# JuliaLinearAlgebra/AlgebraicMultigrid.jl

Measured on AMD Instinct MI355X. Metric: V-cycle unknowns/sec + fine-level SpMV GB/s (% HBM peak), 3-D Poisson 256^3, higher is better.
Workload: dtype f64

## Files before the change

algebraicmultigrid.jl_amd/csrc/hip/amghip.hip:

```cpp
#include "amghip_internal.hpp"
#include "gs_schedule.hpp"
#include "csr_ops.hpp"
#include "chebyshev.hpp"
#include "gmres_kernels.hpp"
#include "pcg_block_kernels.hpp"
#include "dist_pcg_kernels.hpp"

namespace {

constexpr int64_t kGraphAutoRows = 65536;

struct Level {
  int64_t n = 0, nc = 0;
  amgh_csr A, S, P, R;
  bool has_S = false;
  amgh_smoother_t pre{}, post{};
  real *res = nullptr, *cx = nullptr, *cb = nullptr, *tmp = nullptr;
  real* cheb_d = nullptr;
  ChebSide cheb[2];
  const ChebSide& cheb_of(const amgh_smoother_t& s) const { return &s == &post ? cheb[1] : cheb[0]; }
  real* il = nullptr;
  amgh_csr* smat() { return has_S ? &S : &A; }
  amgh_csr Pp, Rp;
  bool lo_ok = false;
// ... 1289 lines not shown
      }
      if (L->Pp.cc.ccol) {
        double t_il = 0, t_st = 0;
        RC_TRY(hipMemsetAsync(L->cx, 0, sizeof(real) * nc * bs, h->stream) == hipSuccess ? AMGH_OK : -1001);
        RC_TRY(hipMemsetAsync(L->res, 0, sizeof(real) * n * bs, h->stream) == hipSuccess ? AMGH_OK : -1001);
        RC_TRY(timed([&] { return il_apply(bs, true, L->Pp.rowptr, L->Pp.col, L->Pp.val, n, L->cx, nc, nc, L->il, L->res, n, h->stream, &L->Pp.cc); }, &t_il));
        RC_TRY(timed([&] { return raw_apply(M_ADD, L->Pp.rowptr, L->Pp.col, L->Pp.val, n, L->cx, nc, nullptr, 0, L->res, n, h->stream, bs, &L->Pp.cc); }, &t_st));
        L->p_stream = t_st < 0.95 * t_il;
        if (getenv("AMGH_VERBOSE")) fprintf(stderr, "[amghip] n=%lld prolongation of %d columns: interleaved %.3f ms, column by column %.3f ms\n", (long long)n, bs, t_il / 2, t_st / 2);
      }
    }
  }
  if (h->nrhs == 1)
    for (Level* L : h->levels) {
      if (!L->lo_ok || !L->Rp.rowptr || L->Rp.nrows < (1 << 18)) continue;
      if (hipMemsetAsync(L->res, 0, sizeof(real) * L->n, h->stream) != hipSuccess) return -1001;
      double ms[2] = {0, 0};
      int rc = AMGH_OK;
      for (int v = 0; v < 2 && rc == AMGH_OK; ++v) {
        L->Rp.xcd_map = v == 1;
        rc = csr_apply(&L->Rp, M_SPMV, L->res, nullptr, L->cb, h->stream, 1);
        if (rc == AMGH_OK && hipEventRecord(h->t0, h->stream) != hipSuccess) rc = -1001;
        for (int r = 0; r < 4 && rc == AMGH_OK; ++r) rc = csr_apply(&L->Rp, M_SPMV, L->res, nullptr, L->cb, h->stream, 1);
        float t = 0.f;
        if (rc == AMGH_OK && (hipEventRecord(h->t1, h->stream) != hipSuccess || hipEventSynchronize(h->t1) != hipSuccess ||
                              hipEventElapsedTime(&t, h->t0, h->t1) != hipSuccess)) rc = -1001;
        ms[v] = t;
      }
      L->Rp.xcd_map = false;
      RC_TRY(rc);
      L->Rp.xcd_map = ms[1] < 0.93 * ms[0];
      if (getenv("AMGH_VERBOSE")) fprintf(stderr, "[amghip] n=%lld restriction: %.3f ms, XCD-contiguous %.3f ms -> %s\n", (long long)L->n, ms[0] / 4, ms[1] / 4, L->Rp.xcd_map ? "XCD-contiguous" : "plain");
    }
  if (gs_trim() && g_stream_code && g_trim_coded) {
    HIP_TRY(hipStreamSynchronize(h->stream));
    for (Level* L : h->levels) {
      for (amgh_csr* M : {&L->Rp, &L->Pp})
        if (M->cc.ccol && M->col && M->val) {
          hipFree(M->col); hipFree(M->val); M->col = nullptr; M->val = nullptr;
          M->bytes -= M->nnz * kEntB;
        }
      amgh_csr* S = L->smat();
      GsSchedule* g = S->gs;
      if (L->lo_cc.ccol && g && g->bw.on && g->bw.flow.on && !g->bw.rec && g->segs.empty() && !g->mf && !g->mb && g->col && g->val) {
        hipFree(g->col); hipFree(g->val); g->col = nullptr; g->val = nullptr;
        int64_t freed = g->nnz * kEntB;
        if (L->lo_val) { hipFree(L->lo_val); L->lo_val = nullptr; }
        g->csr_bytes -= freed; g->bytes -= freed; S->bytes -= freed;
      }
    }
  }
  for (size_t l = 0; l + 1 < h->levels.size(); ++l)
    if (h->levels[l]->coarse_lo) RC_TRY(gs_ensure_cols(h->levels[l + 1]->smat(), h->nrhs, h->stream));
  const int64_t n = fine_n(h);
  if (h->levels.empty()) { RC_TRY(dev_alloc(&h->res_final, n * h->nrhs)); ws += kRealB * n * h->nrhs; }
  RC_TRY(dev_alloc(&h->partial, kRedBlocks));
  RC_TRY(dev_alloc(&h->scal, 8));
  RC_TRY(dev_alloc(&h->x0, n * h->nrhs));
  RC_TRY(dev_alloc(&h->b0, n * h->nrhs));
  ws += 2 * kRealB * n * h->nrhs;
  h->ws_bytes = ws;
  if (h->graph_auto && !h->levels.empty() && getenv("AMGH_GRAPH_AUTO") && getenv("AMGH_GRAPH_AUTO")[0] == '1') {
    int64_t widest = 0;
    for (Level* L : h->levels) widest = std::max(widest, L->n);
    h->use_graph = widest <= kGraphAutoRows;
  }
// ... 504 lines not shown
}

int amgh_csr_create(amgh_csr_t** opp, int device, int64_t nrows, int64_t ncols, const int32_t* rowptr,
                    const int32_t* col, const real* val) {
  if (!opp) return AMGH_EINVAL;
  *opp = nullptr;
  int ndev = 0;
  HIP_TRY(hipGetDeviceCount(&ndev));
  if (device < 0 || device >= ndev) return AMGH_EINVAL;
  HIP_TRY(hipSetDevice(device));
  amgh_csr* op = new amgh_csr;
  int rc = csr_upload(op, device, nrows, ncols, rowptr, col, val);
  if (rc != AMGH_OK) { csr_free(op); delete op; return rc; }
  *opp = op;
  return AMGH_OK;
}
void amgh_csr_destroy(amgh_csr_t* op) {
  if (!op) return;
  hipSetDevice(op->device);
  csr_free(op);
  delete op;
}
int amgh_csr_prepare(amgh_csr_t* op, int jacobi, int gs) {
  if (!op) return AMGH_EINVAL;
  HIP_TRY(hipSetDevice(op->device));
  if (jacobi) RC_TRY(csr_ensure_diag(op, nullptr));
  if (gs) RC_TRY(csr_ensure_gs(op));
  HIP_TRY(hipDeviceSynchronize());
  return AMGH_OK;
}
int amgh_csr_spmv_d(amgh_csr_t* op, const real* x_d, real* y_d, void* stream) {
  if (!op || !x_d || !y_d) return AMGH_EINVAL;
  HIP_TRY(hipSetDevice(op->device));
  return csr_apply(op, M_SPMV, x_d, nullptr, y_d, (hipStream_t)stream);
}
int amgh_csr_residual_d(amgh_csr_t* op, const real* x_d, const real* b_d, real* r_d, void* stream) {
  if (!op || !x_d || !b_d || !r_d) return AMGH_EINVAL;
  HIP_TRY(hipSetDevice(op->device));
  return csr_apply(op, M_RESID, x_d, b_d, r_d, (hipStream_t)stream);
}
int amgh_csr_spmv_add_d(amgh_csr_t* op, const real* x_d, real* y_d, void* stream) {
  if (!op || !x_d || !y_d) return AMGH_EINVAL;
  HIP_TRY(hipSetDevice(op->device));
  return csr_apply(op, M_ADD, x_d, nullptr, y_d, (hipStream_t)stream);
}
int amgh_csr_jacobi_d(amgh_csr_t* op, double omega, const real* xin_d, const real* b_d, real* xout_d,
                      void* stream) {
  if (!op || !xin_d || !b_d || !xout_d || xin_d == xout_d) return AMGH_EINVAL;
  HIP_TRY(hipSetDevice(op->device));
  return csr_jacobi(op, omega, xin_d, b_d, xout_d, (hipStream_t)stream);
}
int amgh_csr_gs_d(amgh_csr_t* op, int backward, double omega, int is_sor, real* x_d, const real* b_d,
                  void* stream) {
  if (!op || !x_d || !b_d) return AMGH_EINVAL;
  HIP_TRY(hipSetDevice(op->device));
  return csr_gs_sweep(op, backward != 0, is_sor != 0, omega, x_d, b_d, (hipStream_t)stream);
}
int amgh_csr_gs_ex_d(amgh_csr_t* op, int backward, double omega, int is_sor, real* x_d, const real* b_d,
                     void* stream, int flags) {
  if (!op || !x_d || !b_d || (flags & ~AMGH_GS_REUSE_B)) return AMGH_EINVAL;
  HIP_TRY(hipSetDevice(op->device));
  return csr_gs_sweep(op, backward != 0, is_sor != 0, omega, x_d, b_d, (hipStream_t)stream, true, true, 1, false,
                      (flags & AMGH_GS_REUSE_B) != 0);
}

int amgh_gather_d(int device, int64_t n, const int32_t* idx_d, const real* src_d, real* dst_d, void* stream) {
  if (n < 0 || (n > 0 && (!idx_d || !src_d || !dst_d)) || n >= INT32_MAX) return AMGH_EINVAL;
  if (n == 0) return AMGH_OK;
  HIP_TRY(hipSetDevice(device));
  hipLaunchKernelGGL(gather_perm_kernel, dim3(grid_for(n)), dim3(256), 0, (hipStream_t)stream, src_d, idx_d, dst_d,
                     (int)n, (int64_t)0, (int64_t)0);
  HIP_TRY(hipGetLastError());
  return AMGH_OK;
}

int amgh_dot_d(int device, int64_t n, const real* x_d, const real* y_d, real* scratch_d, real* out,
// ... 400 lines not shown
  else if (!strcmp(name, "gs_bw_rows")) *value = g_gs_bw_rows;
  else if (!strcmp(name, "gs_bw_chain")) *value = g_gs_bw_chain;
  else if (!strcmp(name, "gs_bw_flow")) *value = g_gs_bw_flow;
  else if (!strcmp(name, "gs_bw_spin")) *value = g_gs_bw_spin;
  else if (!strcmp(name, "gs_bw_nc")) *value = g_gs_bw_nc;
  else if (!strcmp(name, "gs_bw_nrhs")) *value = g_gs_bw_nrhs;
  else if (!strcmp(name, "gs_bw_skip_pub")) *value = g_gs_bw_skip_pub;
  else if (!strcmp(name, "gs_bw_two_min_rows")) *value = g_gs_bw_two_min_rows;
  else if (!strcmp(name, "gs_flow_xzero")) *value = g_gs_flow_xzero;
  else if (!strcmp(name, "gs_bw_dict")) *value = g_gs_bw_dict;
  else if (!strcmp(name, "gs_bw_inorder")) *value = g_gs_bw_inorder;
  else if (!strcmp(name, "stream_code")) *value = g_stream_code;
  else if (!strcmp(name, "gs_bw_relay")) *value = g_gs_bw_relay;
  else if (!strcmp(name, "rhs_il")) *value = g_rhs_il;
  else if (!strcmp(name, "jacobi_zero")) *value = g_jacobi_zero;
  else if (!strcmp(name, "gs_ept")) *value = g_gs_ept;
  else if (!strcmp(name, "gs_merge")) *value = g_gs_merge;
  else if (!strcmp(name, "gs_coarse_lo")) *value = g_gs_coarse_lo;
  else if (!strcmp(name, "gs_dense_tri")) *value = g_gs_dense_tri;
  else if (!strcmp(name, "gs_dense_blk")) *value = g_gs_dense_blk;
  else if (!strcmp(name, "gs_bigslot")) *value = g_gs_bigslot;
  else if (!strcmp(name, "gs_super")) *value = g_gs_super;
  else if (!strcmp(name, "gs_block_pipe")) *value = g_gs_block_pipe;
  else return AMGH_EINVAL;
  return AMGH_OK;
}

int amgh_debug_set_perm_io(int on) {
  g_gs_flow_perm_io = on != 0;
  ++g_sched_epoch;
  return AMGH_OK;
}
int amgh_debug_get_perm_io(void) { return g_gs_flow_perm_io; }
int amgh_debug_perm_io_sweeps(int which) { return (which == 0 || which == 1) ? (int)(g_perm_io_sweeps[which] & 0x7fffffffu) : -1; }

int amgh_debug_chain_timing(int enable, unsigned long long* out8) {
  if (enable && !g_chain_tim) {
    HIP_TRY(hipMalloc((void**)&g_chain_tim, 8 * sizeof(unsigned long long)));
    HIP_TRY(hipMemset(g_chain_tim, 0, 8 * sizeof(unsigned long long)));
  }
  if (out8 && g_chain_tim) {
    HIP_TRY(hipDeviceSynchronize());
    HIP_TRY(hipMemcpy(out8, g_chain_tim, 8 * sizeof(unsigned long long), hipMemcpyDeviceToHost));
    HIP_TRY(hipMemset(g_chain_tim, 0, 8 * sizeof(unsigned long long)));
  }
  if (!enable && g_chain_tim) { hipFree(g_chain_tim); g_chain_tim = nullptr; }
  return AMGH_OK;
}

int amgh_profile_enable(amgh_t* h, int on) {
  if (!h) return AMGH_EINVAL;
  h->profile = on != 0;
  return AMGH_OK;
}
int amgh_profile_read(amgh_t* h, double* out, int reset) {
  if (!h || !out) return AMGH_EINVAL;
  RC_TRY(prof_flush(h));
  const int L1 = (int)h->levels.size() + 1;
  if ((int)h->prof_ms.size() != AMGH_T_COUNT * L1) h->prof_ms.assign(AMGH_T_COUNT * L1, 0.0);
  std::copy(h->prof_ms.begin(), h->prof_ms.end(), out);
  if (reset) std::fill(h->prof_ms.begin(), h->prof_ms.end(), 0.0);
  return AMGH_OK;
}
int amgh_set_use_graph(amgh_t* h, int on) {
  if (!h) return AMGH_EINVAL;
  h->use_graph = on != 0;
// ... 11 lines not shown
```

algebraicmultigrid.jl_amd/csrc/hip/amghip_internal.hpp:

```cpp
#pragma once
#include "amghip_kernels.hpp"
#include "gs_blocks.hpp"
#include "gs_flow.hpp"

#include <algorithm>
#include <chrono>
#include <cmath>
#include <cstdio>
#include <cstring>
#include <atomic>
#include <mutex>
#include <string>
#include <system_error>
#include <thread>
#include <utility>
#include <vector>

#include "../../../include/amghip.h"

using namespace amgh;

#define HIP_TRY(expr)                                   \
  do {                                                  \
    hipError_t e_ = (expr);                             \
// ... 265 lines not shown
      hipFree(o->sp_rowptr); hipFree(o->sp_col); hipFree(o->sp_val);
      *o = Outer();
    }
    hipFree(dti_f); if (dti_b != dti_f) hipFree(dti_b);
    dti_f = dti_b = nullptr;
    for (Tri* t : {&dtri_f, &dtri_b}) { hipFree(t->rowptr); hipFree(t->col); hipFree(t->val); *t = Tri(); }
    hipFree(blk_diag); blk_diag = nullptr;
    hipFree(blk_s); blk_s = nullptr;
    hipFree(wcol); hipFree(wval); hipFree(slot_row); hipFree(wmeta); wcol = slot_row = nullptr; wval = nullptr; wmeta = nullptr;
    hipFree(scol); hipFree(sval); hipFree(schunk); scol = nullptr; sval = nullptr; schunk = nullptr;
    hipFree(ww_rec); ww_rec = nullptr;
    hipFree(wq_rec); wq_rec = nullptr;
    hipFree(xil); xil = nullptr; xil_cap = 0; xil_cols = 0;
    hipFree(bw.blocks); hipFree(bw.rec); hipFree(bw.ext_col);
    hipFree(bw.dep_ptr); hipFree(bw.dep); hipFree(bw.sdep_ptr); hipFree(bw.sdep); hipFree(bw.flags); hipFree(bw.head);
    hipFree(bw.flow.fd); hipFree(bw.flow.srec); hipFree(bw.flow.aux); hipFree(bw.flow.fl_mb); hipFree(bw.flow.fl_slot); hipFree(bw.flow.mbox);
    hipFree(bw.flow.xaux); hipFree(bw.flow.xfl_mb); hipFree(bw.flow.xfl_slot); hipFree(bw.flow.xlist);
    hipFree(bw.flow.crec); hipFree(bw.flow.dict); hipFree(bw.flow.dict_ent);
    bw = Bw();
    hipFree(d_lvl_ptr); hipFree(rowptr); hipFree(col); hipFree(val);
    hipFree(perm); hipFree(dpos); if (!diag_shared) hipFree(diag);
    hipFree(rowmeta); hipFree(desc); hipFree(bp); hipFree(xp); hipFree(permx);
    d_lvl_ptr = rowptr = col = perm = dpos = nullptr; val = diag = bp = xp = nullptr; rowmeta = desc = nullptr; permx = nullptr;
  }
};

}

#include "dev_scan.hpp"

struct CodedCols {
  uint32_t* ccol = nullptr; real* vtab = nullptr; int n = 0;
  int64_t bytes = 0;
  void free_dev() { hipFree(ccol); hipFree(vtab); ccol = nullptr; vtab = nullptr; n = 0; bytes = 0; }
};

struct amgh_csr {
  CodedCols cc;
  bool cc_tried = false;
  bool xcd_map = false;
  int device = 0;
  int64_t nrows = 0, ncols = 0, nnz = 0;
  int32_t* rowptr = nullptr;
  int32_t* col = nullptr;
  real* val = nullptr;
  int32_t* dpos = nullptr;
  real* diag = nullptr;
  GsSchedule* gs = nullptr;
  int gs_nrhs_hint = 0;
  uint32_t pipe_epoch = 0; const void* pipe_rmbox = nullptr; int pipe_grid = 0;
  int64_t bytes = 0;
};

namespace {

int g_gs_block_pipe = 1;
int g_gs_super = 8;
int g_gs_coarse_lo = 1;
int g_gs_bigslot = 1;
int g_gs_merge = 16;
int g_jacobi_zero = 1;
int g_rhs_il = 1;
int g_gs_tiny = 1;
int g_gs_wave_quad = 1;
int g_gs_bw = 1;
int g_gs_bw_rows = 512;
int g_gs_bw_flow = 1;
int g_gs_bw_spin = 0;
int g_gs_bw_skip_pub = -1;
int g_gs_bw_nc = -1;
int g_gs_bw_nrhs = 1;
int g_gs_bw_chain = 1;
int g_stream_code = 1;
int g_trim_coded = 1;
int g_gs_bw_inorder = 0;
int g_gs_bw_dict = 1;
int g_gs_bw_relay = 3;
int g_gs_flow_xzero = 1;
int g_gs_flow_perm_io = 1;
unsigned int g_perm_io_sweeps[2] = {0, 0};
int g_gs_bw_two_min_rows = 200000;
int g_gs_sell = 1;
int g_gs_lean = -1;
int g_gs_ept = 0;
int g_gs_lpr = 0;
int g_gs_il = 1;
int g_pcg_fused = 1;
int g_tail_dense_rows = 6144;
int g_tail_dense = 1;
int g_gs_dense_blk = 4096;
int g_gs_dense_tri = 1;
int g_gs_block_inverse = 1;

std::atomic<unsigned long long> g_sched_epoch{0};

unsigned long long* g_chain_tim = nullptr;

constexpr int kChainWidth = 1024;

__global__ void find_diag_kernel(const int32_t* rowptr, const int32_t* col, const real* val, int n,
                                 int32_t* dpos, real* diag) {
  const int i = blockIdx.x * blockDim.x + threadIdx.x;
  if (i >= n) return;
  int dp = -1;
  real d = 0.0;
  for (int j = rowptr[i]; j < rowptr[i + 1]; ++j)
// ... 52 lines not shown
```

algebraicmultigrid.jl_amd/csrc/hip/amghip_kernels.hpp:

```cpp
#pragma once
#include <hip/hip_runtime.h>
#include <stdint.h>

#ifndef AMGH_REAL
#define AMGH_REAL double
#endif

namespace amgh {

using real = AMGH_REAL;

constexpr int kWave = 64;
constexpr int kThreads = 256;
constexpr int kNumXcd = 8;

enum StreamMode : int {
  M_SPMV = 0,
  M_RESID = 1,
  M_ADD = 2,
  M_JACOBI = 3,
  M_GS = 4,
  M_SOR = 5,
  M_CHEB1 = 6,
  M_CHEB = 7
// ... 48 lines not shown
typedef int i2_t __attribute__((ext_vector_type(2)));
typedef int i4_t __attribute__((ext_vector_type(4)));

template <int CTRL>
__device__ __forceinline__ double dpp_move(double v) {
  int lo = __double2loint(v), hi = __double2hiint(v);
  lo = __builtin_amdgcn_update_dpp(0, lo, CTRL, 0xf, 0xf, false);
  hi = __builtin_amdgcn_update_dpp(0, hi, CTRL, 0xf, 0xf, false);
  return __hiloint2double(hi, lo);
}
template <int CTRL>
__device__ __forceinline__ float dpp_move(float v) {
  return __int_as_float(__builtin_amdgcn_update_dpp(0, __float_as_int(v), CTRL, 0xf, 0xf, false));
}
template <int W>
__device__ __forceinline__ real tree_add(real acc) {
#pragma unroll
  for (int w = 1; w < W; w <<= 1) {
    if (w == 1) acc += dpp_move<0xB1>(acc);
    else if (w == 2) acc += dpp_move<0x4E>(acc);
    else if (w == 4) acc += dpp_move<0x141>(acc);
    else if (w == 8) acc += dpp_move<0x140>(acc);
    else acc += __shfl_xor(acc, w, kWave);
  }
  return acc;
}

template <bool NT, class T>
__device__ __forceinline__ T ld_stream(const T* p) {
  if (NT) return __builtin_nontemporal_load(p);
  return *p;
}

template <int THREADS_, int ROWS_, int LDS_NNZ_, int VEC_, bool NT_, bool XCD_>
struct StreamCfg {
  static constexpr int THREADS = THREADS_;
  static constexpr int ROWS = ROWS_;
  static constexpr int RPT = (ROWS_ + THREADS_ - 1) / THREADS_;
  static constexpr int LDS_NNZ = LDS_NNZ_;
  static constexpr int VEC = VEC_;
  static constexpr bool NT = NT_;
  static constexpr bool XCD = XCD_;
};

template <bool SKIPD>
__device__ __forceinline__ real seq_sum(const real* s_prod, int lo, int hi, int c0, int dp, real acc) {
  int j = lo;
  for (; j + 8 <= hi; j += 8) {
    real p[8];
#pragma unroll
    for (int e = 0; e < 8; ++e) p[e] = s_prod[skew(j + e - c0)];
#pragma unroll
    for (int e = 0; e < 8; ++e) {
      if (SKIPD) acc = (j + e != dp) ? acc + p[e] : acc;
      else acc += p[e];
    }
  }
  for (; j < hi; ++j) {
    const real p = s_prod[skew(j - c0)];
    if (SKIPD) acc = (j != dp) ? acc + p : acc;
    else acc += p;
  }
  return acc;
}

template <int MODE, class CFG, bool CODED = false>
__global__ __launch_bounds__(CFG::THREADS) void csr_stream_kernel(StreamArgs a) {
  constexpr int T = CFG::THREADS, RPT = CFG::RPT, LDSN = CFG::LDS_NNZ, VEC = CFG::VEC;
  constexpr bool NT = CFG::NT;
  static_assert(!CODED || (VEC == 4 && T >= kCodeMax), "the value-coded variant is the big-operator configuration's");
  __shared__ real s_tab[CODED ? kCodeMax : 1];
  if (CODED) {
    if ((int)threadIdx.x < a.vtab_n) s_tab[threadIdx.x] = a.vtab[threadIdx.x];
    __syncthreads();
  }
  constexpr bool SK = CFG::ROWS > 64;
  __shared__ real s_prod[LDSN + (LDSN >> 5) + 2];
  int bid, cv;
  multi_column_block(a.ncolv, bid, cv);
  if (cv > 0) {
    a.x += cv * a.ldx;
    a.y += cv * a.ldy;
    if (a.b) a.b += cv * a.ldb;
    if (MODE >= M_CHEB1) a.d += cv * a.ldd;
  }

  const int nrows = a.row_end - a.row_begin;
  const int nb = (nrows + CFG::ROWS - 1) / CFG::ROWS;
  const int lb = CFG::XCD ? xcd_block(bid, nb) : bid;
  if (lb >= nb) return;
  const int r0 = a.row_begin + lb * CFG::ROWS;
  const int r1 = min(r0 + CFG::ROWS, a.row_end);
  const int tid = threadIdx.x;

  int rs[RPT], re[RPT], dp[RPT], gi[RPT];
  real acc[RPT], gd[RPT], gb[RPT];
#pragma unroll
  for (int q = 0; q < RPT; ++q) {
    const int r = r0 + tid + q * T;
    gi[q] = 0; gd[q] = 0.0; gb[q] = 0.0;
    if (tid + q * T < CFG::ROWS && r < r1) {
      rs[q] = a.rowptr[r];
      re[q] = a.rowptr[r + 1];
      dp[q] = kSkipDiag<MODE> ? a.dpos[r] : -1;
      if (kLevelRows<MODE>) {
        gi[q] = a.perm ? a.perm[r] : r;
        gd[q] = a.diag[r];
        gb[q] = a.b[r];
      }
    } else {
      rs[q] = re[q] = 0;
      dp[q] = -1;
    }
    acc[q] = 0.0;
  }
  const int p0 = a.rowptr[r0];
  const int p1 = a.rowptr[r1];

  for (int c0 = p0; c0 < p1; c0 += LDSN) {
    const int c1 = min(c0 + LDSN, p1);
    if (VEC == 1) {
      for (int k = c0 + tid; k < c1; k += T) {
        const real v = ld_stream<NT>(a.val + k);
        const int c = ld_stream<NT>(a.col + k);
        s_prod[lidx<SK>(k - c0)] = v * a.x[c];
      }
    } else {
      const int a0 = c0 & ~(VEC - 1);
      for (int k = a0 + VEC * tid; k < c1; k += VEC * T) {
        if (k >= c0 && k + VEC <= c1) {
          real v[VEC];
          int c[VEC];
          if (VEC == 2) {
            const d2_t vv = ld_stream<NT>((const d2_t*)(a.val + k));
            const i2_t cc = ld_stream<NT>((const i2_t*)(a.col + k));
            v[0] = vv.x; v[1] = vv.y; c[0] = cc.x; c[1] = cc.y;
          } else if (CODED) {
            const u4_t cc = ld_stream<NT>((const u4_t*)(a.ccol + k));
            c[0] = (int)(cc.x & ((1u << kCodeBits) - 1)); c[1] = (int)(cc.y & ((1u << kCodeBits) - 1));
            c[VEC - 2] = (int)(cc.z & ((1u << kCodeBits) - 1)); c[VEC - 1] = (int)(cc.w & ((1u << kCodeBits) - 1));
            v[0] = s_tab[cc.x >> kCodeBits]; v[1] = s_tab[cc.y >> kCodeBits];
            v[VEC - 2] = s_tab[cc.z >> kCodeBits]; v[VEC - 1] = s_tab[cc.w >> kCodeBits];
          } else {
            const d2_t v0 = ld_stream<NT>((const d2_t*)(a.val + k));
            const d2_t v1 = ld_stream<NT>((const d2_t*)(a.val + k + 2));
            const i4_t cc = ld_stream<NT>((const i4_t*)(a.col + k));
            v[0] = v0.x; v[1] = v0.y; v[VEC - 2] = v1.x; v[VEC - 1] = v1.y;
            c[0] = cc.x; c[1] = cc.y; c[VEC - 2] = cc.z; c[VEC - 1] = cc.w;
          }
          real xv[VEC];
#pragma unroll
          for (int e = 0; e < VEC; ++e) xv[e] = a.x[c[e]];
#pragma unroll
          for (int e = 0; e < VEC; ++e) s_prod[lidx<SK>(k + e - c0)] = v[e] * xv[e];
        } else {
#pragma unroll
          for (int e = 0; e < VEC; ++e) {
            const int kk = k + e;
// ... 1728 lines not shown
```

algebraicmultigrid.jl_amd/csrc/hip/csr_ops.hpp:

```cpp
#pragma once
#include <atomic>

namespace {


template <int MODE, class CFG = DefaultCfg, bool CODED = false>
int launch_stream(const StreamArgs& a0, hipStream_t st, int ncolv = 1) {
  const int nrows = a0.row_end - a0.row_begin;
  if (nrows <= 0) return AMGH_OK;
  StreamArgs a = a0;
  a.ncolv = ncolv;
  const int nb = (nrows + CFG::ROWS - 1) / CFG::ROWS;
  const int64_t grid = (CFG::XCD || ncolv > 1) ? (int64_t)((nb + kNumXcd - 1) / kNumXcd) * kNumXcd * ncolv : nb;
  hipLaunchKernelGGL((csr_stream_kernel<MODE, CFG, CODED>), dim3((unsigned)grid), dim3(CFG::THREADS), 0, st, a);
  HIP_TRY(hipGetLastError());
  return AMGH_OK;
}

constexpr int kGsBlockTarget = 256;
constexpr int kGsMinRows = 4;
constexpr int kGsNnzPerWg = 256;
template <int MODE>
int launch_gs_level(const StreamArgs& a, int rows, hipStream_t st, int ncolv = 1) {
  const int width = a.row_end - a.row_begin;
  const int avg16 = std::max(16, rows);
  rows = 256;
  while (rows > kGsMinRows && (int64_t)rows * avg16 > (int64_t)kGsNnzPerWg * 16) rows >>= 1;
  while (rows > kGsMinRows && width / rows < kGsBlockTarget && (int64_t)rows * avg16 > 16 * 64) rows >>= 1;
  switch (rows) {
    case 4: return launch_stream<MODE, StreamCfg<256, 4, 2048, 1, false, false>>(a, st, ncolv);
    case 8: return launch_stream<MODE, StreamCfg<256, 8, 2048, 1, false, false>>(a, st, ncolv);
    case 16: return launch_stream<MODE, StreamCfg<256, 16, 2048, 1, false, false>>(a, st, ncolv);
    case 32: return launch_stream<MODE, StreamCfg<256, 32, 2048, 1, false, false>>(a, st, ncolv);
    case 64: return launch_stream<MODE, StreamCfg<256, 64, 2048, 1, false, false>>(a, st, ncolv);
    case 128: return launch_stream<MODE, StreamCfg<256, 128, 2048, 1, false, false>>(a, st, ncolv);
    default: return launch_stream<MODE, StreamCfg<256, 256, 2048, 2, false, false>>(a, st, ncolv);
  }
}

using SmallCfg = StreamCfg<256, 64, 4096, 2, false, false>;
#ifndef AMGH_CODED_CFG
#define AMGH_CODED_CFG 1024, 1024, 8192, 4
#endif
using CodedCfg = StreamCfg<AMGH_CODED_CFG, false, false>;
template <int MODE>
int launch_stream_sized(const StreamArgs& a, hipStream_t st, int ncolv, bool xcd = false) {
  if (a.row_end - a.row_begin < (1 << 18)) return launch_stream<MODE, SmallCfg>(a, st, ncolv);
  if constexpr (MODE == M_SPMV) {
    if (xcd && ncolv == 1) {
      if (a.ccol && (g_stream_code || !a.col)) return launch_stream<MODE, StreamCfg<1024, 1024, 8192, 4, false, true>, true>(a, st, ncolv);
      return launch_stream<MODE, StreamCfg<1024, 1024, 8192, 4, false, true>>(a, st, ncolv);
    }
  }
  if (a.ccol && (g_stream_code || !a.col)) return launch_stream<MODE, CodedCfg, true>(a, st, ncolv);
  return launch_stream<MODE>(a, st, ncolv);
}

typedef std::conditional<sizeof(real) == 8, unsigned long long, unsigned int>::type rbits_t;
__device__ __forceinline__ rbits_t real_bits(real v) { rbits_t b; __builtin_memcpy(&b, &v, sizeof(real)); return b; }
constexpr int kCodeMiss = 4096;
__device__ __forceinline__ int code_find(const rbits_t* tab, int ntab, rbits_t v) {
  int lo = 0, hi = ntab;
  while (lo < hi) { const int mid = (lo + hi) >> 1; if (tab[mid] < v) lo = mid + 1; else hi = mid; }
  return (lo < ntab && tab[lo] == v) ? lo : -1;
}
__global__ void code_probe_kernel(const real* val, int64_t nnz, const real* tab, int ntab, unsigned* miss_cnt, real* miss) {
  __shared__ rbits_t s_tab[kCodeMax];
  if ((int)threadIdx.x < ntab) s_tab[threadIdx.x] = real_bits(tab[threadIdx.x]);
  __syncthreads();
  for (int64_t k = (int64_t)blockIdx.x * blockDim.x + threadIdx.x; k < nnz; k += (int64_t)gridDim.x * blockDim.x) {
    const real v = val[k];
    if (code_find(s_tab, ntab, real_bits(v)) >= 0) continue;
    if (__hip_atomic_load(miss_cnt, __ATOMIC_RELAXED, __HIP_MEMORY_SCOPE_AGENT) >= (unsigned)kCodeMiss) continue;
    const unsigned i = atomicAdd(miss_cnt, 1u);
    if (i < (unsigned)kCodeMiss) miss[i] = v;
  }
}
__global__ void code_encode_kernel(const int32_t* col, const real* val, int64_t nnz, const real* tab, int ntab, uint32_t* ccol) {
  __shared__ rbits_t s_tab[kCodeMax];
  if ((int)threadIdx.x < ntab) s_tab[threadIdx.x] = real_bits(tab[threadIdx.x]);
  __syncthreads();
  for (int64_t k = (int64_t)blockIdx.x * blockDim.x + threadIdx.x; k < nnz; k += (int64_t)gridDim.x * blockDim.x)
    ccol[k] = (uint32_t)col[k] | ((uint32_t)code_find(s_tab, ntab, real_bits(val[k])) << kCodeBits);
}
int code_values(const int32_t* col, const real* val, int64_t nrows, int64_t ncols, int64_t nnz, CodedCols* out, hipStream_t st) {
  if (!g_stream_code || out->ccol || nrows < (1 << 18) || ncols > ((int64_t)1 << kCodeBits) || nnz <= 0 || !col || !val) return AMGH_OK;
  unsigned* d_cnt = nullptr; real *d_miss = nullptr, *d_tab = nullptr;
  RC_TRY(dev_alloc(&d_cnt, 1));
  int rc = dev_alloc(&d_miss, kCodeMiss);
  if (rc == AMGH_OK) rc = dev_alloc(&d_tab, kCodeMax);
  std::vector<rbits_t> tab;
  std::vector<real> miss((size_t)kCodeMiss);
  bool ok = rc == AMGH_OK;
  for (int pass = 0; ok && pass < 8; ++pass) {
    const int64_t span = pass == 0 ? std::min<int64_t>(nnz, 1 << 20) : nnz;
    const int ntab = (int)tab.size();
    if (hipMemsetAsync(d_cnt, 0, 4, st) != hipSuccess) { rc = -1001; break; }
    if (ntab > 0) {
      std::vector<real> tv((size_t)ntab);
      for (int i = 0; i < ntab; ++i) std::memcpy(&tv[(size_t)i], &tab[(size_t)i], sizeof(real));
      if (hipMemcpyAsync(d_tab, tv.data(), sizeof(real) * (size_t)ntab, hipMemcpyHostToDevice, st) != hipSuccess) { rc = -1001; break; }
      if (hipStreamSynchronize(st) != hipSuccess) { rc = -1001; break; }
    }
    hipLaunchKernelGGL(code_probe_kernel, dim3((unsigned)std::min<int64_t>((span + 255) / 256, 8192)), dim3(256), 0, st, val, span, (const real*)d_tab, ntab, d_cnt, d_miss);
    unsigned cnt = 0;
    if (hipMemcpyAsync(&cnt, d_cnt, 4, hipMemcpyDeviceToHost, st) != hipSuccess || hipStreamSynchronize(st) != hipSuccess) { rc = -1001; break; }
    if (cnt == 0) { if (pass > 0) break; else continue; }
    const unsigned got = std::min<unsigned>(cnt, (unsigned)kCodeMiss);
    if (hipMemcpy(miss.data(), d_miss, sizeof(real) * got, hipMemcpyDeviceToHost) != hipSuccess) { rc = -1001; break; }
    for (unsigned i = 0; i < got; ++i) { rbits_t b; std::memcpy(&b, &miss[i], sizeof(real)); tab.push_back(b); }
    std::sort(tab.begin(), tab.end());
    tab.erase(std::unique(tab.begin(), tab.end()), tab.end());
    if ((int)tab.size() > kCodeMax) ok = false;
    if (pass == 7) ok = false;
  }
  if (rc == AMGH_OK && ok && !tab.empty()) {
    std::vector<real> tv(tab.size());
    for (size_t i = 0; i < tab.size(); ++i) std::memcpy(&tv[i], &tab[i], sizeof(real));
    rc = dev_alloc(&out->ccol, nnz + 4);
    if (rc == AMGH_OK) rc = dev_alloc(&out->vtab, kCodeMax);
    if (rc == AMGH_OK && hipMemcpyAsync(d_tab, tv.data(), sizeof(real) * tv.size(), hipMemcpyHostToDevice, st) != hipSuccess) rc = -1001;
    if (rc == AMGH_OK && hipMemcpyAsync(out->vtab, tv.data(), sizeof(real) * tv.size(), hipMemcpyHostToDevice, st) != hipSuccess) rc = -1001;
    if (rc == AMGH_OK) {
      hipLaunchKernelGGL(code_encode_kernel, dim3((unsigned)std::min<int64_t>((nnz + 255) / 256, 8192)), dim3(256), 0, st, col, val, nnz, (const real*)d_tab, (int)tab.size(), out->ccol);
      if (hipGetLastError() != hipSuccess || hipStreamSynchronize(st) != hipSuccess) rc = -1001;
    }
    if (rc == AMGH_OK) { out->n = (int)tab.size(); out->bytes = nnz * 4 + kCodeMax * kRealB; }
    else out->free_dev();
  }
  hipFree(d_cnt); hipFree(d_miss); hipFree(d_tab);
  if (rc == AMGH_ENOMEM) { (void)hipGetLastError(); out->free_dev(); return AMGH_OK; }
  return rc;
}

int csr_apply(const amgh_csr* op, int mode, const real* x, const real* b, real* y, hipStream_t st,
              int ncolv = 1) {
  StreamArgs a{};
  a.rowptr = op->rowptr; a.col = op->col; a.val = op->val;
  a.ccol = op->cc.ccol; a.vtab = op->cc.vtab; a.vtab_n = op->cc.n;
  a.x = x; a.y = y; a.b = b;
  a.row_begin = 0; a.row_end = (int32_t)op->nrows;
  a.ldx = op->ncols; a.ldy = op->nrows; a.ldb = op->nrows;
  switch (mode) {
    case M_SPMV: return launch_stream_sized<M_SPMV>(a, st, ncolv, op->xcd_map);
    case M_RESID: return launch_stream_sized<M_RESID>(a, st, ncolv);
    case M_ADD: return launch_stream_sized<M_ADD>(a, st, ncolv);
  }
  return AMGH_EINVAL;
}

int csr_jacobi(amgh_csr* op, real omega, const real* xin, const real* b, real* xout, hipStream_t st,
               int ncolv = 1) {
  RC_TRY(csr_ensure_diag(op, st));
  StreamArgs a{};
  a.rowptr = op->rowptr; a.col = op->col; a.val = op->val;
  a.x = xin; a.y = xout; a.b = b; a.dpos = op->dpos; a.diag = op->diag; a.omega = omega;
  a.row_begin = 0; a.row_end = (int32_t)op->nrows;
  a.ldx = op->ncols; a.ldy = op->nrows; a.ldb = op->nrows;
  return launch_stream_sized<M_JACOBI>(a, st, ncolv);
}

int csr_jacobi_zero(amgh_csr* op, real omega, const real* b, real* xout, hipStream_t st, int ncolv = 1) {
  RC_TRY(csr_ensure_diag(op, st));
  if (op->nrows > 0)
    hipLaunchKernelGGL(jacobi_zero_kernel, dim3((unsigned)std::min<int64_t>((op->nrows + 255) / 256, 1 << 20), ncolv), dim3(256), 0, st,
                       b, (const real*)op->diag, xout, (int64_t)op->nrows, omega, (int64_t)op->nrows, (int64_t)op->nrows);
  HIP_TRY(hipGetLastError());
  return AMGH_OK;
}

int csr_chebyshev(amgh_csr* op, real c1, real c2, bool first, const real* xin, const real* b, real* d, real* xout, hipStream_t st,
                  int ncolv = 1) {
  RC_TRY(csr_ensure_diag(op, st));
  StreamArgs a{};
  a.rowptr = op->rowptr; a.col = op->col; a.val = op->val;
  a.ccol = op->cc.ccol; a.vtab = op->cc.vtab; a.vtab_n = op->cc.n;
  a.x = xin; a.y = xout; a.b = b; a.diag = op->diag; a.d = d; a.c1 = c1; a.c2 = c2;
  a.row_begin = 0; a.row_end = (int32_t)op->nrows;
  a.ldx = op->ncols; a.ldy = op->nrows; a.ldb = op->nrows; a.ldd = op->nrows;
// ... 94 lines not shown
  return g->segs.size() == 1 && g->segs[0].chain && g->segs[0].l0 == 0 && g->segs[0].l1 == g->nlev;
}
template <int T>
int launch_chain_tiny_t(const ChainArgs& c, bool sor, int n, int nnz, int nlev, hipStream_t st, int ncolv) {
  if (sor) hipLaunchKernelGGL((gs_chain_tiny_kernel<true, T>), dim3(ncolv), dim3(T), 0, st, c, n, nnz, nlev);
  else hipLaunchKernelGGL((gs_chain_tiny_kernel<false, T>), dim3(ncolv), dim3(T), 0, st, c, n, nnz, nlev);
  HIP_TRY(hipGetLastError());
  return AMGH_OK;
}
int launch_chain_tiny(const ChainArgs& c, bool sor, int threads, int n, int nnz, int nlev, hipStream_t st, int ncolv) {
  switch (threads) {
    case 64: return launch_chain_tiny_t<64>(c, sor, n, nnz, nlev, st, ncolv);
    case 256: return launch_chain_tiny_t<256>(c, sor, n, nnz, nlev, st, ncolv);
    default: return launch_chain_tiny_t<1024>(c, sor, n, nnz, nlev, st, ncolv);
  }
}
int launch_chain(const ChainArgs& c, bool sor, bool ldsx, int threads, int nx, hipStream_t st, int ncolv) {
  switch (threads) {
    case 64: return launch_chain_t<64, 4>(c, sor, ldsx, nx, st, ncolv);
    case 256: return launch_chain_t<256, 4>(c, sor, ldsx, nx, st, ncolv);
    default: return launch_chain_t<1024, 4>(c, sor, ldsx, nx, st, ncolv);
  }
}

int raw_apply(int mode, const int32_t* rowptr, const int32_t* col, const real* val, int64_t nrows, const real* x,
              int64_t ldx, const real* b, int64_t ldb, real* y, int64_t ldy, hipStream_t st, int ncolv, const CodedCols* cc = nullptr) {
  StreamArgs a{};
  a.rowptr = rowptr; a.col = col; a.val = val;
  if (cc) { a.ccol = cc->ccol; a.vtab = cc->vtab; a.vtab_n = cc->n; }
  a.x = x; a.y = y; a.b = b;
  a.row_begin = 0; a.row_end = (int32_t)nrows;
  a.ldx = ldx; a.ldy = ldy; a.ldb = ldb;
  switch (mode) {
    case M_SPMV: return launch_stream_sized<M_SPMV>(a, st, ncolv);
    case M_RESID: return launch_stream_sized<M_RESID>(a, st, ncolv);
    case M_ADD: return launch_stream_sized<M_ADD>(a, st, ncolv);
  }
  return AMGH_EINVAL;
}

template <int BS>
int il_apply_t(bool add, const int32_t* rowptr, const int32_t* col, const real* val, int64_t nrows, const real* x, int64_t nx,
               int64_t ldx, real* il, real* y, int64_t ldy, hipStream_t st, const CodedCols* cc) {
  if (nx > 0)
    hipLaunchKernelGGL((to_interleaved_kernel<BS>), dim3((unsigned)((nx + 63) / 64)), dim3(256), 0, st, x, ldx, il, nx);
  const int64_t threads = nrows * BS;
  if (threads > 0) {
    const unsigned grid = (unsigned)((threads + 255) / 256);
    if (cc && cc->ccol && (g_stream_code || !col)) {
      if (add) hipLaunchKernelGGL((csr_il_kernel<true, BS, true>), dim3(grid), dim3(256), 0, st, rowptr, (const int32_t*)cc->ccol, (const real*)cc->vtab, nrows, (const real*)il, y, ldy, cc->n);
      else hipLaunchKernelGGL((csr_il_kernel<false, BS, true>), dim3(grid), dim3(256), 0, st, rowptr, (const int32_t*)cc->ccol, (const real*)cc->vtab, nrows, (const real*)il, y, ldy, cc->n);
    } else
    if (add) hipLaunchKernelGGL((csr_il_kernel<true, BS>), dim3(grid), dim3(256), 0, st, rowptr, col, val, nrows, (const real*)il, y, ldy);
    else hipLaunchKernelGGL((csr_il_kernel<false, BS>), dim3(grid), dim3(256), 0, st, rowptr, col, val, nrows, (const real*)il, y, ldy);
  }
  HIP_TRY(hipGetLastError());
  return AMGH_OK;
}
int il_apply(int bs, bool add, const int32_t* rowptr, const int32_t* col, const real* val, int64_t nrows, const real* x,
             int64_t nx, int64_t ldx, real* il, real* y, int64_t ldy, hipStream_t st, const CodedCols* cc = nullptr) {
  switch (bs) {
    case 2: return il_apply_t<2>(add, rowptr, col, val, nrows, x, nx, ldx, il, y, ldy, st, cc);
    case 4: return il_apply_t<4>(add, rowptr, col, val, nrows, x, nx, ldx, il, y, ldy, st, cc);
    case 8: return il_apply_t<8>(add, rowptr, col, val, nrows, x, nx, ldx, il, y, ldy, st, cc);
    case 16: return il_apply_t<16>(add, rowptr, col, val, nrows, x, nx, ldx, il, y, ldy, st, cc);
  }
  return AMGH_EUNSUPPORTED;
}
inline bool il_block(int bs) { return g_rhs_il && (bs == 2 || bs == 4 || bs == 8 || bs == 16); }
// ... 523 lines not shown
```

include/amghip.h:

```cpp
#ifndef AMGHIP_H
#define AMGHIP_H

#include <stdint.h>

#ifdef __cplusplus
extern "C" {
#endif

#ifndef AMGH_REAL
#define AMGH_REAL double
#endif
typedef AMGH_REAL amgh_real;

typedef struct amgh_handle amgh_t;
typedef struct amgh_csr amgh_csr_t;

#define AMGH_OK 0
#define AMGH_EINVAL (-2)
#define AMGH_ESTATE (-3)
#define AMGH_ENOMEM (-4)
#define AMGH_EUNSUPPORTED (-5)

enum { AMGH_SMOOTH_NONE = 0, AMGH_SMOOTH_GS = 1, AMGH_SMOOTH_JACOBI = 2, AMGH_SMOOTH_SOR = 3, AMGH_SMOOTH_CHEBYSHEV = 4 };
enum { AMGH_SWEEP_FORWARD = 0, AMGH_SWEEP_BACKWARD = 1, AMGH_SWEEP_SYMMETRIC = 2 };
// ... 201 lines not shown
int amgh_dev_sync(int device);
void* amgh_stream(amgh_t* h);

int amgh_timer_begin(amgh_t* h);
int amgh_timer_end(amgh_t* h, double* ms);
int amgh_bench_op(amgh_t* h, int level, int which, int reps, int warmup, double* avg_ms);

int amgh_profile_enable(amgh_t* h, int on);
int amgh_profile_read(amgh_t* h, double* out, int reset);

int amgh_debug_chain_timing(int enable, unsigned long long* out8);
int amgh_debug_merged_sweep_host(int64_t nrows, int64_t ncols, const int32_t* rowptr, const int32_t* col,
                                 const amgh_real* val, int m, int backward, double omega ,
                                 amgh_real* x, const amgh_real* b);

int amgh_debug_bw_sweep_host(int64_t nrows, const int32_t* rowptr, const int32_t* col, const amgh_real* val, int target_rows,
                             int backward, double omega, amgh_real* x, const amgh_real* b, int64_t* stats4);

int amgh_debug_bw_dict_sweep_host(int64_t nrows, const int32_t* rowptr, const int32_t* col, const amgh_real* val, int target_rows,
                                  int backward, amgh_real* x, const amgh_real* b, int64_t* stats5);

int amgh_debug_bw_poll_giveups(const amgh_t* h, int l);

int amgh_debug_bw_mode(const amgh_t* h, int l);
int amgh_debug_bw_dict(const amgh_t* h, int l);
int amgh_debug_bw_late(const amgh_t* h, int l);
int amgh_debug_coded_ops(const amgh_t* h, int l);

int amgh_debug_set_tunable(const char* name, int value);
int amgh_debug_get_tunable(const char* name, int* value);
int amgh_debug_set_perm_io(int on);
int amgh_debug_get_perm_io(void);
int amgh_debug_perm_io_sweeps(int which);

int amgh_set_use_graph(amgh_t* h, int on);

#ifdef __cplusplus
}
#endif
#endif
```

Before: 1.214 billion.

## Add lane-consecutive coded-column load variants for stream SpMV, autotuned per operator

Adds two alternative ways for the value-coded CSR stream kernel to load packed column/value codes. One uses lane-consecutive 4-byte loads, the other uses 16-byte loads followed by a cross-lane transpose via ds_bpermute, so the products land in the same consecutive-lane order as the first. At setup, the residual, restriction and prolongation operators with at least 2^18 rows are timed under each variant, and a variant is kept only if it beats the default by more than the run-to-run spread. The aim is better memory coalescing of the index stream, at the cost of extra setup timing work, more kernel instantiations and an extra debug knob.

```diff
diff --git a/algebraicmultigrid.jl_amd/csrc/hip/amghip.hip b/algebraicmultigrid.jl_amd/csrc/hip/amghip.hip
--- a/algebraicmultigrid.jl_amd/csrc/hip/amghip.hip
+++ b/algebraicmultigrid.jl_amd/csrc/hip/amghip.hip
@@ -1345,6 +1345,53 @@
       L->Rp.xcd_map = ms[1] < 0.93 * ms[0];
       if (getenv("AMGH_VERBOSE")) fprintf(stderr, "[amghip] n=%lld restriction: %.3f ms, XCD-contiguous %.3f ms -> %s\n", (long long)L->n, ms[0] / 4, ms[1] / 4, L->Rp.xcd_map ? "XCD-contiguous" : "plain");
     }
+  if (h->nrhs == 1 && g_stream_lanes == 1 && g_stream_code) {
+    for (Level* L : h->levels) {
+      GsSchedule* g = L->smat()->gs;
+      struct Cand { CodedCols* cc; int mode; int64_t nrows, ncols; const char* name; };
+      const Cand cands[3] = {{&L->lo_cc, M_RESID, L->n, g ? (int64_t)g->ncols : 0, "residual"},
+                             {&L->Rp.cc, M_SPMV, L->Rp.nrows, L->Rp.ncols, "restriction"},
+                             {&L->Pp.cc, M_ADD, L->Pp.nrows, L->Pp.ncols, "prolongation"}};
+      for (const Cand& c : cands) {
+        if (!L->lo_ok || !g || !c.cc->ccol || c.nrows < (1 << 18)) continue;
+        real *tx = nullptr, *ty = nullptr, *tb = nullptr;
+        int rc = dev_alloc(&tx, c.ncols);
+        if (rc == AMGH_OK) rc = dev_alloc(&ty, c.nrows);
+        if (rc == AMGH_OK && c.mode == M_RESID) rc = dev_alloc(&tb, c.nrows);
+        if (rc == AMGH_ENOMEM) { (void)hipGetLastError(); hipFree(tx); hipFree(ty); hipFree(tb); continue; }
+        if (rc == AMGH_OK && (hipMemsetAsync(tx, 0x3f, sizeof(real) * c.ncols, h->stream) != hipSuccess ||
+                              hipMemsetAsync(ty, 0x3f, sizeof(real) * c.nrows, h->stream) != hipSuccess ||
+                              (tb && hipMemsetAsync(tb, 0x3f, sizeof(real) * c.nrows, h->stream) != hipSuccess))) rc = -1001;
+        auto run = [&]() -> int {
+          if (c.cc == &L->Rp.cc) return csr_apply(&L->Rp, M_SPMV, tx, nullptr, ty, h->stream, 1);
+          if (c.mode == M_RESID) return raw_apply(M_RESID, g->rowptr, g->col, L->lo_val ? L->lo_val : g->val, c.nrows, tx, c.ncols, tb, c.nrows, ty, c.nrows, h->stream, 1, c.cc);
+          return raw_apply(M_ADD, L->Pp.rowptr, L->Pp.col, L->Pp.val, c.nrows, tx, c.ncols, nullptr, 0, ty, c.nrows, h->stream, 1, c.cc);
+        };
+        double mean[3] = {0, 0, 0}, lo[3] = {1e30, 1e30, 1e30}, hi[3] = {0, 0, 0};
+        for (int rep = 0; rep < 3 && rc == AMGH_OK; ++rep)
+          for (int v = 0; v < 3 && rc == AMGH_OK; ++v) {
+            c.cc->lanes = v;
+            rc = run();
+            if (rc == AMGH_OK && hipEventRecord(h->t0, h->stream) != hipSuccess) rc = -1001;
+            for (int r = 0; r < 4 && rc == AMGH_OK; ++r) rc = run();
+            float t = 0.f;
+            if (rc == AMGH_OK && (hipEventRecord(h->t1, h->stream) != hipSuccess || hipEventSynchronize(h->t1) != hipSuccess ||
+                                  hipEventElapsedTime(&t, h->t0, h->t1) != hipSuccess)) rc = -1001;
+            mean[v] += t / 12.0; lo[v] = std::min(lo[v], t / 4.0); hi[v] = std::max(hi[v], t / 4.0);
+          }
+        c.cc->lanes = 0;
+        hipFree(tx); hipFree(ty); hipFree(tb);
+        RC_TRY(rc);
+        const int best = mean[2] < mean[1] ? 2 : 1;
+        const double spread = std::max(hi[0] - lo[0], hi[best] - lo[best]);
+        if (mean[best] + spread < mean[0] && mean[best] < 0.98 * mean[0]) c.cc->lanes = best;
+        if (getenv("AMGH_VERBOSE"))
+          fprintf(stderr, "[amghip] n=%lld %s: shipped %.4f ms (%.4f - %.4f), lane-consecutive 4 x 4 B %.4f (%.4f - %.4f), transposed %.4f (%.4f - %.4f) -> %s\n",
+                  (long long)L->n, c.name, mean[0], lo[0], hi[0], mean[1], lo[1], hi[1], mean[2], lo[2], hi[2],
+                  c.cc->lanes == 1 ? "4 x 4 B" : c.cc->lanes == 2 ? "transposed" : "shipped");
+      }
+    }
+  }
   if (gs_trim() && g_stream_code && g_trim_coded) {
     HIP_TRY(hipStreamSynchronize(h->stream));
     for (Level* L : h->levels) {
@@ -1915,16 +1962,19 @@
 int amgh_csr_spmv_d(amgh_csr_t* op, const real* x_d, real* y_d, void* stream) {
   if (!op || !x_d || !y_d) return AMGH_EINVAL;
   HIP_TRY(hipSetDevice(op->device));
+  if (g_stream_lanes >= 2) RC_TRY(csr_ensure_coded(op, (hipStream_t)stream));
   return csr_apply(op, M_SPMV, x_d, nullptr, y_d, (hipStream_t)stream);
 }
 int amgh_csr_residual_d(amgh_csr_t* op, const real* x_d, const real* b_d, real* r_d, void* stream) {
   if (!op || !x_d || !b_d || !r_d) return AMGH_EINVAL;
   HIP_TRY(hipSetDevice(op->device));
+  if (g_stream_lanes >= 2) RC_TRY(csr_ensure_coded(op, (hipStream_t)stream));
   return csr_apply(op, M_RESID, x_d, b_d, r_d, (hipStream_t)stream);
 }
 int amgh_csr_spmv_add_d(amgh_csr_t* op, const real* x_d, real* y_d, void* stream) {
   if (!op || !x_d || !y_d) return AMGH_EINVAL;
   HIP_TRY(hipSetDevice(op->device));
+  if (g_stream_lanes >= 2) RC_TRY(csr_ensure_coded(op, (hipStream_t)stream));
   return csr_apply(op, M_ADD, x_d, nullptr, y_d, (hipStream_t)stream);
 }
 int amgh_csr_jacobi_d(amgh_csr_t* op, double omega, const real* xin_d, const real* b_d, real* xout_d,
@@ -2391,6 +2441,12 @@
   return AMGH_OK;
 }
 int amgh_debug_get_perm_io(void) { return g_gs_flow_perm_io; }
+int amgh_debug_set_stream_lanes(int mode) {
+  if (mode < 0 || mode > 7 || mode == 4 || mode == 5) return AMGH_EINVAL;
+  g_stream_lanes = mode;
+  return AMGH_OK;
+}
+int amgh_debug_stream_lanes_launches(void) { return (int)(g_stream_lanes_launches & 0x7fffffffu); }
 int amgh_debug_perm_io_sweeps(int which) { return (which == 0 || which == 1) ? (int)(g_perm_io_sweeps[which] & 0x7fffffffu) : -1; }
 
 int amgh_debug_chain_timing(int enable, unsigned long long* out8) {
diff --git a/algebraicmultigrid.jl_amd/csrc/hip/amghip_internal.hpp b/algebraicmultigrid.jl_amd/csrc/hip/amghip_internal.hpp
--- a/algebraicmultigrid.jl_amd/csrc/hip/amghip_internal.hpp
+++ b/algebraicmultigrid.jl_amd/csrc/hip/amghip_internal.hpp
@@ -321,7 +321,8 @@
 struct CodedCols {
   uint32_t* ccol = nullptr; real* vtab = nullptr; int n = 0;
   int64_t bytes = 0;
-  void free_dev() { hipFree(ccol); hipFree(vtab); ccol = nullptr; vtab = nullptr; n = 0; bytes = 0; }
+  int lanes = 0;
+  void free_dev() { hipFree(ccol); hipFree(vtab); ccol = nullptr; vtab = nullptr; n = 0; bytes = 0; lanes = 0; }
 };
 
 struct amgh_csr {
@@ -361,6 +362,8 @@
 int g_gs_bw_nrhs = 1;
 int g_gs_bw_chain = 1;
 int g_stream_code = 1;
+int g_stream_lanes = 1;
+unsigned int g_stream_lanes_launches = 0;
 int g_trim_coded = 1;
 int g_gs_bw_inorder = 0;
 int g_gs_bw_dict = 1;
diff --git a/algebraicmultigrid.jl_amd/csrc/hip/amghip_kernels.hpp b/algebraicmultigrid.jl_amd/csrc/hip/amghip_kernels.hpp
--- a/algebraicmultigrid.jl_amd/csrc/hip/amghip_kernels.hpp
+++ b/algebraicmultigrid.jl_amd/csrc/hip/amghip_kernels.hpp
@@ -104,6 +104,25 @@
   return *p;
 }
 
+__device__ __forceinline__ void lane_transpose(u4_t c, int lane, unsigned (&w)[4]) {
+  const unsigned in[4] = {c.x, c.y, c.z, c.w};
+  const bool r1 = (lane >> 4) & 1, r2 = (lane >> 5) & 1;
+  unsigned t[4], v[4], g[4];
+#pragma unroll
+  for (int m = 0; m < 4; ++m) t[m] = r1 ? in[(m + 1) & 3] : in[m];
+#pragma unroll
+  for (int m = 0; m < 4; ++m) v[m] = r2 ? t[(m + 2) & 3] : t[m];
+  const int e = lane & 3, q = lane >> 2;
+#pragma unroll
+  for (int m = 0; m < 4; ++m) g[m] = (unsigned)__builtin_amdgcn_ds_bpermute(4 * (16 * ((e - m) & 3) + q), (int)v[m]);
+  const bool e1 = e & 1, e2 = (e >> 1) & 1;
+#pragma unroll
+  for (int m = 0; m < 4; ++m) t[m] = e1 ? g[(m + 1) & 3] : g[m];
+#pragma unroll
+  for (int m = 0; m < 4; ++m) v[m] = e2 ? t[(m + 2) & 3] : t[m];
+  w[0] = v[0]; w[1] = v[3]; w[2] = v[2]; w[3] = v[1];
+}
+
 template <int THREADS_, int ROWS_, int LDS_NNZ_, int VEC_, bool NT_, bool XCD_>
 struct StreamCfg {
   static constexpr int THREADS = THREADS_;
@@ -136,11 +155,12 @@
   return acc;
 }
 
-template <int MODE, class CFG, bool CODED = false>
+template <int MODE, class CFG, bool CODED = false, int LANEK = 0>
 __global__ __launch_bounds__(CFG::THREADS) void csr_stream_kernel(StreamArgs a) {
   constexpr int T = CFG::THREADS, RPT = CFG::RPT, LDSN = CFG::LDS_NNZ, VEC = CFG::VEC;
   constexpr bool NT = CFG::NT;
   static_assert(!CODED || (VEC == 4 && T >= kCodeMax), "the value-coded variant is the big-operator configuration's");
+  static_assert(LANEK == 0 || (CODED && LANEK <= 2 && T % kWave == 0), "lane-consecutive entries: value-coded variant only");
   __shared__ real s_tab[CODED ? kCodeMax : 1];
   if (CODED) {
     if ((int)threadIdx.x < a.vtab_n) s_tab[threadIdx.x] = a.vtab[threadIdx.x];
@@ -196,6 +216,34 @@
         const real v = ld_stream<NT>(a.val + k);
         const int c = ld_stream<NT>(a.col + k);
         s_prod[lidx<SK>(k - c0)] = v * a.x[c];
+      }
+    } else if (LANEK) {
+      const int a0 = c0 & ~3;
+      const int lane = tid & (kWave - 1);
+      constexpr unsigned kColMask = (1u << kCodeBits) - 1;
+      for (int base = a0 + 4 * kWave * __builtin_amdgcn_readfirstlane(tid / kWave); base < c1; base += 4 * T) {
+        if (base >= c0 && base + 4 * kWave <= c1) {
+          unsigned w[4];
+          if (LANEK == 1) {
+#pragma unroll
+            for (int j = 0; j < 4; ++j) w[j] = ld_stream<NT>(a.ccol + base + kWave * j + lane);
+          } else {
+            lane_transpose(ld_stream<NT>((const u4_t*)(a.ccol + base + 4 * lane)), lane, w);
+          }
+          real v[4], xv[4];
+#pragma unroll
+          for (int j = 0; j < 4; ++j) v[j] = s_tab[w[j] >> kCodeBits];
+#pragma unroll
+          for (int j = 0; j < 4; ++j) xv[j] = a.x[(int)(w[j] & kColMask)];
+#pragma unroll
+          for (int j = 0; j < 4; ++j) s_prod[lidx<SK>(base + kWave * j + lane - c0)] = v[j] * xv[j];
+        } else {
+#pragma unroll
+          for (int j = 0; j < 4; ++j) {
+            const int kk = base + kWave * j + lane;
+            if (kk >= c0 && kk < c1) { const unsigned w = a.ccol[kk]; s_prod[lidx<SK>(kk - c0)] = s_tab[w >> kCodeBits] * a.x[w & kColMask]; }
+          }
+        }
       }
     } else {
       const int a0 = c0 & ~(VEC - 1);
diff --git a/algebraicmultigrid.jl_amd/csrc/hip/csr_ops.hpp b/algebraicmultigrid.jl_amd/csrc/hip/csr_ops.hpp
--- a/algebraicmultigrid.jl_amd/csrc/hip/csr_ops.hpp
+++ b/algebraicmultigrid.jl_amd/csrc/hip/csr_ops.hpp
@@ -4,7 +4,7 @@
 namespace {
 
 
-template <int MODE, class CFG = DefaultCfg, bool CODED = false>
+template <int MODE, class CFG = DefaultCfg, bool CODED = false, int LANEK = 0>
 int launch_stream(const StreamArgs& a0, hipStream_t st, int ncolv = 1) {
   const int nrows = a0.row_end - a0.row_begin;
   if (nrows <= 0) return AMGH_OK;
@@ -12,8 +12,9 @@
   a.ncolv = ncolv;
   const int nb = (nrows + CFG::ROWS - 1) / CFG::ROWS;
   const int64_t grid = (CFG::XCD || ncolv > 1) ? (int64_t)((nb + kNumXcd - 1) / kNumXcd) * kNumXcd * ncolv : nb;
-  hipLaunchKernelGGL((csr_stream_kernel<MODE, CFG, CODED>), dim3((unsigned)grid), dim3(CFG::THREADS), 0, st, a);
-  HIP_TRY(hipGetLastError());
+  hipLaunchKernelGGL((csr_stream_kernel<MODE, CFG, CODED, LANEK>), dim3((unsigned)grid), dim3(CFG::THREADS), 0, st, a);
+  HIP_TRY(hipGetLastError());
+  if (LANEK) ++g_stream_lanes_launches;
   return AMGH_OK;
 }
 
@@ -43,16 +44,29 @@
 #define AMGH_CODED_CFG 1024, 1024, 8192, 4
 #endif
 using CodedCfg = StreamCfg<AMGH_CODED_CFG, false, false>;
+template <int MODE, class CFG>
+int launch_stream_coded(const StreamArgs& a, hipStream_t st, int ncolv, int lk) {
+  if constexpr (MODE == M_SPMV || MODE == M_RESID || MODE == M_ADD) {
+    if (lk == 1) return launch_stream<MODE, CFG, true, 1>(a, st, ncolv);
+    if (lk == 2) return launch_stream<MODE, CFG, true, 2>(a, st, ncolv);
+  }
+  return launch_stream<MODE, CFG, true>(a, st, ncolv);
+}
 template <int MODE>
-int launch_stream_sized(const StreamArgs& a, hipStream_t st, int ncolv, bool xcd = false) {
-  if (a.row_end - a.row_begin < (1 << 18)) return launch_stream<MODE, SmallCfg>(a, st, ncolv);
+int launch_stream_sized(const StreamArgs& a, hipStream_t st, int ncolv, bool xcd = false, int lanes = 0) {
+  const bool coded = a.ccol && (g_stream_code || !a.col);
+  int lk = 0;
+  if (coded && ncolv == 1 && (MODE == M_SPMV || MODE == M_RESID || MODE == M_ADD))
+    lk = g_stream_lanes == 1 ? lanes : g_stream_lanes >= 2 ? 1 + (g_stream_lanes & 1) : 0;
+  if (a.row_end - a.row_begin < (1 << 18) && !(lk && g_stream_lanes >= 2)) return launch_stream<MODE, SmallCfg>(a, st, ncolv);
+  if (lk && g_stream_lanes >= 6) xcd = true;
   if constexpr (MODE == M_SPMV) {
     if (xcd && ncolv == 1) {
-      if (a.ccol && (g_stream_code || !a.col)) return launch_stream<MODE, StreamCfg<1024, 1024, 8192, 4, false, true>, true>(a, st, ncolv);
+      if (coded) return launch_stream_coded<MODE, StreamCfg<1024, 1024, 8192, 4, false, true>>(a, st, ncolv, lk);
       return launch_stream<MODE, StreamCfg<1024, 1024, 8192, 4, false, true>>(a, st, ncolv);
     }
   }
-  if (a.ccol && (g_stream_code || !a.col)) return launch_stream<MODE, CodedCfg, true>(a, st, ncolv);
+  if (coded) return launch_stream_coded<MODE, CodedCfg>(a, st, ncolv, lk);
   return launch_stream<MODE>(a, st, ncolv);
 }
 
@@ -84,7 +98,7 @@
     ccol[k] = (uint32_t)col[k] | ((uint32_t)code_find(s_tab, ntab, real_bits(val[k])) << kCodeBits);
 }
 int code_values(const int32_t* col, const real* val, int64_t nrows, int64_t ncols, int64_t nnz, CodedCols* out, hipStream_t st) {
-  if (!g_stream_code || out->ccol || nrows < (1 << 18) || ncols > ((int64_t)1 << kCodeBits) || nnz <= 0 || !col || !val) return AMGH_OK;
+  if (!g_stream_code || out->ccol || (nrows < (1 << 18) && g_stream_lanes < 2) || ncols > ((int64_t)1 << kCodeBits) || nnz <= 0 || !col || !val) return AMGH_OK;
   unsigned* d_cnt = nullptr; real *d_miss = nullptr, *d_tab = nullptr;
   RC_TRY(dev_alloc(&d_cnt, 1));
   int rc = dev_alloc(&d_miss, kCodeMiss);
@@ -142,9 +156,9 @@
   a.row_begin = 0; a.row_end = (int32_t)op->nrows;
   a.ldx = op->ncols; a.ldy = op->nrows; a.ldb = op->nrows;
   switch (mode) {
-    case M_SPMV: return launch_stream_sized<M_SPMV>(a, st, ncolv, op->xcd_map);
-    case M_RESID: return launch_stream_sized<M_RESID>(a, st, ncolv);
-    case M_ADD: return launch_stream_sized<M_ADD>(a, st, ncolv);
+    case M_SPMV: return launch_stream_sized<M_SPMV>(a, st, ncolv, op->xcd_map, op->cc.lanes);
+    case M_RESID: return launch_stream_sized<M_RESID>(a, st, ncolv, false, op->cc.lanes);
+    case M_ADD: return launch_stream_sized<M_ADD>(a, st, ncolv, false, op->cc.lanes);
   }
   return AMGH_EINVAL;
 }
@@ -305,9 +319,9 @@
   a.row_begin = 0; a.row_end = (int32_t)nrows;
   a.ldx = ldx; a.ldy = ldy; a.ldb = ldb;
   switch (mode) {
-    case M_SPMV: return launch_stream_sized<M_SPMV>(a, st, ncolv);
-    case M_RESID: return launch_stream_sized<M_RESID>(a, st, ncolv);
-    case M_ADD: return launch_stream_sized<M_ADD>(a, st, ncolv);
+    case M_SPMV: return launch_stream_sized<M_SPMV>(a, st, ncolv, false, cc ? cc->lanes : 0);
+    case M_RESID: return launch_stream_sized<M_RESID>(a, st, ncolv, false, cc ? cc->lanes : 0);
+    case M_ADD: return launch_stream_sized<M_ADD>(a, st, ncolv, false, cc ? cc->lanes : 0);
   }
   return AMGH_EINVAL;
 }
diff --git a/include/amghip.h b/include/amghip.h
--- a/include/amghip.h
+++ b/include/amghip.h
@@ -257,6 +257,8 @@
 int amgh_debug_set_perm_io(int on);
 int amgh_debug_get_perm_io(void);
 int amgh_debug_perm_io_sweeps(int which);
+int amgh_debug_set_stream_lanes(int mode);
+int amgh_debug_stream_lanes_launches(void);
 
 int amgh_set_use_graph(amgh_t* h, int on);
 
```

Result: no change. 1.203 billion (-0.9%).
